# ruiminshen/yolo2-pytorch

Hardware: AMD Instinct MI355X
Metric: images/sec (416x416) train+detect, Darknet-19 YOLOv2: value = TRAIN step, batch 64 per GPU (configs[2]) at every N; detect (configs[1]) = roofline.detect_images_per_sec (higher is better)
Workload: dtype f32; 1 GPU; Darknet-19 YOLOv2 20-class train 416x416 batch-64/GPU: fwd + region loss + bwd + SGD (BASELINE configs[2]); classes=20, global_batch=64, parallelism=single GPU, weights=random-init seed 0 (bench_data.randomize)

## Files before the change

### include/yolo2_hip.h

```cpp
#ifndef YOLO2_HIP_H
#define YOLO2_HIP_H

#include <stdint.h>

#ifdef __cplusplus
extern "C" {
#endif

#define Y2_OK 0
#define Y2_EINVAL (-1)
#define Y2_EALIGN (-2)
#define Y2_ENOSUP (-3)

#define Y2_STATS_REPL 32

typedef void* y2_stream_t;

int y2_abi_version(void);
const char* y2_build_info(void);


int y2_pack_weight(const float* w, float* dst, int Cout, int Cin, int ksize, int mode, y2_stream_t stream);

#define Y2_PREP_FPROP 0
// ... 153 lines not shown
                       const float* gt_min, const float* gt_max, const long long* gt_cls, const uint8_t* gt_difficult,
                       int32_t B, int32_t M, int32_t G, int32_t C, float threshold, float min_union, uint8_t* tp, int32_t* cls_num);
int y2_collate_images_host(const uint8_t* src, const int64_t* offset, const int32_t* geom, const float* lut,
                           int32_t B, int32_t H, int32_t W, int32_t flags, float* out);
int y2_warp_affine_images_host(const uint8_t* src, const int64_t* src_offset, const int32_t* src_geom, const double* inv,
                               uint8_t* dst, const int64_t* dst_offset, const int32_t* dst_geom,
                               int32_t B, int32_t max_h, int32_t max_w, int32_t fill);
int y2_collate_jitter_images_host(const uint8_t* src, const int64_t* offset, const int32_t* geom, const int32_t* jitter, const uint8_t* hsv_tab,
                                  const float* lut, int32_t B, int32_t H, int32_t W, int32_t flags, float* out);

int y2_set_deterministic(int on, float* workspace, long long workspace_bytes);
int y2_get_deterministic(void);
int y2_colstats_det(const float* z, long long M, int32_t C, int32_t ld, double* stats, float* workspace, long long workspace_bytes, y2_stream_t stream);

int y2_prof_enable(int on);
int y2_prof_count(void);
int y2_prof_get(int i, char* name, int name_cap, float* ms, double* flops);
int y2_prof_set_tag(int tag);
int y2_prof_get_tag(int i);


int y2_conv_wgrad(const float* x, const float* dz, float* dw, int B, int H, int W, int Cin, int ldx, int Cout, int ldz,
                  int ksize, y2_stream_t stream);

int y2_conv_wgrad_ex(const float* x, const float* dz, float* dw, int B, int Hi, int Wi, int Cin, int ldx, int Cout, int ldz,
                     int ksize, int stride, int pad, y2_stream_t stream);

int y2_conv0_wgrad(const float* x_nchw, const float* dz, float* dw, int B, int H, int W, int Cin, int Cout, int ldz, y2_stream_t stream);

int y2_conv0_wgrad_fused(const float* x_nchw, const float* z, const float* scale, const float* shift, const float* mean, const float* invstd,
                         const float* gamma, float slope, const float* dy_pool, int32_t ldp, const double* sums, float* dw,
                         int32_t B, int32_t H, int32_t W, int32_t Cin, int32_t Cout, int32_t ldz, int32_t has_bn, y2_stream_t stream);

int y2_bn_finalize(const double* stats, double count, const float* gamma, const float* beta,
                   float* running_mean, float* running_var, float momentum, float eps,
                   float* scale, float* shift, float* mean, float* invstd, int C, long long* num_batches_tracked, y2_stream_t stream);

int y2_bn_act_fwd(const float* z, const float* scale, const float* shift, float slope, float* y, float* y_pool,
                  int B, int H, int W, int C, int ldz, int ldy, int coff, int ldp, int poff, int out_mode, y2_stream_t stream);

int y2_bn_act_bwd(const float* z, const float* scale, const float* shift, const float* mean, const float* invstd, const float* gamma,
                  float slope, const float* dy_full, int ldf, int foff, int fmode, const float* dy_pool, int ldp, int poff,
                  double* sums, float* dz, int ldd, int B, int H, int W, int C, int ldz, int has_bn, y2_stream_t stream);

int y2_bn_act_fwd_ex(const float* z, const float* scale, const float* shift, float slope, const float* residual, int ldr, float* y, float* y_pool,
                     int B, int H, int W, int C, int ldz, int ldy, int coff, int ldp, int poff, int out_mode, y2_stream_t stream);
int y2_bn_act_bwd_ex(const float* z, const float* scale, const float* shift, const float* mean, const float* invstd, const float* gamma,
                     float slope, const float* dy_full, int ldf, int foff, int fmode, const float* dy_pool, int ldp, int poff,
                     const float* dy_full2, int ld2, const float* residual, int ldr, float* dres, int lddr,
                     double* sums, float* dz, int ldd, int B, int H, int W, int C, int ldz, int has_bn, y2_stream_t stream);

long long y2_wino6_tiles(int32_t B, int32_t H, int32_t W);
int y2_bn_act_bwd_wino6(const float* z, const float* scale, const float* shift, const float* mean, const float* invstd, const float* gamma,
                        float slope, const float* dy_full, int ldf, int foff, double* sums, float* v6, float* m6, float* dz, int ldd,
                        int B, int H, int W, int C, int ldz, int has_bn, y2_stream_t stream);

int y2_maxpool_bwd(const float* x, const float* dy, const float* dy2, float* dx, int B, int H, int W, int C, int ldx, int ldy, int lddx,
                   int ksize, int stride, int pad, int pad_end, y2_stream_t stream);

int y2_colsum(const float* x, long long M, int C, int ld, double* out, y2_stream_t stream);
int y2_f64_to_f32(const double* src, float* dst, int n, double mul, y2_stream_t stream);

int y2_decode_bwd(const float* iou, const float* center_offset, const float* d_iou, const float* d_center_offset, const float* d_size_norm,
                  const float* d_logits, float* d_feature, int boxes, int C, y2_stream_t stream);

int y2_region_loss_fwd(const float* iou, const float* center_offset, const float* size_norm, const float* logits,
// ... 50 lines not shown
```

### yolo2-pytorch_amd/_hip.py

```python
import ctypes
import os
import subprocess

import torch

_HERE = os.path.dirname(os.path.abspath(__file__))
LIB_PATH = os.environ.get('Y2_LIB') or os.path.join(_HERE, 'csrc', 'libyolo2_hip.so')
_lib = None

c_int, c_float, c_void_p = ctypes.c_int, ctypes.c_float, ctypes.c_void_p


class ConvParams(ctypes.Structure):
    _fields_ = [('x', c_void_p), ('w', c_void_p), ('scale', c_void_p), ('shift', c_void_p),
                ('y', c_void_p), ('y_pool', c_void_p), ('stats', c_void_p),
                ('B', ctypes.c_int32), ('H', ctypes.c_int32), ('W', ctypes.c_int32),
                ('Cin', ctypes.c_int32), ('ldx', ctypes.c_int32), ('Cout', ctypes.c_int32), ('ksize', ctypes.c_int32),
                ('ldy', ctypes.c_int32), ('coff', ctypes.c_int32), ('ldp', ctypes.c_int32), ('poff', ctypes.c_int32),
                ('out_mode', ctypes.c_int32), ('slope', c_float), ('tile', ctypes.c_int32),
                ('workspace', c_void_p), ('workspace_bytes', ctypes.c_int64),
                ('residual', c_void_p), ('ldr', ctypes.c_int32), ('stride', ctypes.c_int32), ('pad_plus1', ctypes.c_int32),
                ('transposed', ctypes.c_int32), ('out_h', ctypes.c_int32), ('out_w', ctypes.c_int32), ('algo', ctypes.c_int32),
                ('w_plane', ctypes.c_int64)]

# ... 35 lines not shown
    'y2_gemm_split_f16': [c_void_p, c_void_p, c_void_p, ctypes.c_longlong, c_int, c_int, c_int, c_int, c_float, c_void_p],
    'y2_gemm_split': [c_void_p, c_void_p, c_void_p, ctypes.c_longlong, c_int, c_int, c_int, c_int, c_void_p],
    'y2_multi': [ctypes.POINTER(MultiItem), c_int, c_void_p],
    'y2_small_dot': [c_void_p, c_void_p, c_int, c_void_p, c_void_p],
    'y2_small_scale': [c_void_p, c_void_p, c_int, c_void_p, c_void_p],
    'y2_unpack_weight_grad': [c_void_p, c_void_p, c_int, c_int, c_int, c_void_p],
    'y2_bn_fold': [c_void_p, c_void_p, c_void_p, c_void_p, c_float, c_void_p, c_void_p, c_int, c_void_p],
    'y2_conv_fwd': [ctypes.POINTER(ConvParams), c_void_p],
    'y2_conv_fwd_workspace_bytes': [ctypes.POINTER(ConvParams)],
    'y2_wino_weight': [c_void_p, c_void_p, c_int, c_int, c_void_p],
    'y2_wino6_weight': [c_void_p, c_void_p, c_int, c_int, c_void_p],
    'y2_opt_sgd': [ctypes.POINTER(OptTensor), c_int, c_float, c_float, c_float, c_float, c_int, c_int, c_void_p],
    'y2_opt_adam': [ctypes.POINTER(OptTensor), c_int, c_float, c_float, c_float, c_float, c_float, c_int, c_void_p],
    'y2_opt_grad_sumsq': [ctypes.POINTER(OptTensor), c_int, c_void_p, c_void_p],
    'y2_opt_clip_grads': [ctypes.POINTER(OptTensor), c_int, c_void_p, c_float, c_void_p],
    'y2_wino_wgrad_workspace_bytes': [c_int, c_int, c_int, c_int, c_int],
    'y2_wino_wgrad_workspace_bytes_ex': [c_int, c_int, c_int, c_int, c_int, c_int],
    'y2_wino_wgrad': [c_void_p, c_void_p, c_void_p, c_int, c_int, c_int, c_int, c_int, c_int, c_int, c_void_p, c_void_p, ctypes.c_longlong, c_void_p],
    'y2_wino_wgrad_ex': [c_void_p, c_void_p, c_void_p, c_int, c_int, c_int, c_int, c_int, c_int, c_int, c_void_p, c_void_p, ctypes.c_longlong, c_int, c_void_p],
    'y2_conv_fwd_batch': [ctypes.POINTER(ConvParams), c_int, c_void_p],
    'y2_conv0_fwd': [c_void_p, c_void_p, c_void_p, c_void_p, c_void_p, c_void_p, c_void_p,
                     c_int, c_int, c_int, c_int, c_int, c_int, c_int, c_float, c_void_p],
    'y2_maxpool2_fwd': [c_void_p, c_void_p, c_int, c_int, c_int, c_int, c_int, c_int, c_void_p],
    'y2_maxpool_fwd': [c_void_p, c_void_p, c_int, c_int, c_int, c_int, c_int, c_int, c_int, c_int, c_int, c_int, c_void_p],
    'y2_nchw_to_nhwc': [c_void_p, c_void_p, c_int, c_int, c_int, c_int, c_int, c_void_p],
    'y2_decode': [c_void_p, c_void_p, c_int, c_int, c_int, c_int, c_int,
                  c_void_p, c_void_p, c_void_p, c_void_p, c_void_p, c_void_p, c_void_p, c_void_p, c_void_p],
    'y2_filter_visible': [c_void_p, c_void_p, c_int, c_int, c_int, c_int, c_float, c_void_p, c_void_p, c_void_p, c_void_p, c_void_p],
    'y2_iou_matrix': [c_void_p, c_void_p, c_void_p, c_void_p, c_int, c_int, c_int, c_float, c_int, c_void_p, c_void_p],
    'y2_iou_pair': [c_void_p, c_void_p, c_void_p, c_void_p, c_int, c_float, c_void_p, c_void_p],
    'y2_conv_wgrad': [c_void_p, c_void_p, c_void_p, c_int, c_int, c_int, c_int, c_int, c_int, c_int, c_int, c_void_p],
    'y2_conv_wgrad_ex': [c_void_p, c_void_p, c_void_p, c_int, c_int, c_int, c_int, c_int, c_int, c_int, c_int, c_int, c_int, c_void_p],
    'y2_conv0_wgrad_fused': [c_void_p] * 7 + [c_float, c_void_p, c_int, c_void_p, c_void_p] + [c_int] * 7 + [c_void_p],
    'y2_conv0_wgrad': [c_void_p, c_void_p, c_void_p, c_int, c_int, c_int, c_int, c_int, c_int, c_void_p],
    'y2_bn_finalize': [c_void_p, ctypes.c_double, c_void_p, c_void_p, c_void_p, c_void_p, c_float, c_float, c_void_p, c_void_p, c_void_p, c_void_p, c_int, c_void_p, c_void_p],
    'y2_bn_act_fwd': [c_void_p, c_void_p, c_void_p, c_float, c_void_p, c_void_p, c_int, c_int, c_int, c_int, c_int, c_int, c_int, c_int, c_int, c_int, c_void_p],
    'y2_bn_act_bwd': [c_void_p, c_void_p, c_void_p, c_void_p, c_void_p, c_void_p, c_float, c_void_p, c_int, c_int, c_int, c_void_p, c_int, c_int,
                      c_void_p, c_void_p, c_int, c_int, c_int, c_int, c_int, c_int, c_int, c_void_p],
    'y2_bn_act_fwd_ex': [c_void_p, c_void_p, c_void_p, c_float, c_void_p, c_int, c_void_p, c_void_p, c_int, c_int, c_int, c_int, c_int, c_int, c_int, c_int, c_int, c_int, c_void_p],
    'y2_bn_act_bwd_ex': [c_void_p, c_void_p, c_void_p, c_void_p, c_void_p, c_void_p, c_float, c_void_p, c_int, c_int, c_int, c_void_p, c_int, c_int,
                         c_void_p, c_int, c_void_p, c_int, c_void_p, c_int,
                         c_void_p, c_void_p, c_int, c_int, c_int, c_int, c_int, c_int, c_int, c_void_p],
    'y2_wino6_tiles': [c_int, c_int, c_int],
    'y2_bn_act_bwd_wino6': [c_void_p, c_void_p, c_void_p, c_void_p, c_void_p, c_void_p, c_float, c_void_p, c_int, c_int, c_void_p, c_void_p, c_void_p, c_void_p, c_int,
                            c_int, c_int, c_int, c_int, c_int, c_int, c_void_p],
    'y2_maxpool_bwd': [c_void_p, c_void_p, c_void_p, c_void_p, c_int, c_int, c_int, c_int, c_int, c_int, c_int, c_int, c_int, c_int, c_int, c_void_p],
    'y2_colsum': [c_void_p, ctypes.c_longlong, c_int, c_int, c_void_p, c_void_p],
    'y2_dwconv_fwd': [c_void_p, c_void_p, c_void_p, c_void_p, c_float, c_void_p, c_void_p, c_int, c_int, c_int, c_int, c_int, c_int, c_int, c_void_p],
    'y2_dwconv_dgrad': [c_void_p, c_void_p, c_void_p, c_int, c_int, c_int, c_int, c_int, c_int, c_int, c_void_p],
    'y2_dwconv_wgrad': [c_void_p, c_void_p, c_void_p, c_void_p, ctypes.c_longlong, c_int, c_int, c_int, c_int, c_int, c_int, c_int, c_void_p],
    'y2_dwconv_wgrad_workspace_bytes': [c_int, c_int, c_int, c_int, c_int],
    'y2_preact_conv1x1_fwd': [c_void_p, c_void_p, c_void_p, c_void_p, c_float, c_void_p, c_void_p, c_float, c_void_p, c_void_p] + [c_int] * 9 + [c_void_p],
    'y2_preact_fwd': [c_void_p, c_void_p, c_void_p, c_float, c_void_p] + [c_int] * 7 + [c_void_p],
    'y2_preact_bwd': [c_void_p, c_void_p, c_void_p, c_float, c_void_p, c_void_p, c_void_p, c_void_p, c_int, c_void_p, c_void_p, c_int, c_int] + [c_int] * 7 + [c_void_p],
    'y2_f64_to_f32': [c_void_p, c_void_p, c_int, ctypes.c_double, c_void_p],
    'y2_decode_bwd': [c_void_p, c_void_p, c_void_p, c_void_p, c_void_p, c_void_p, c_void_p, c_int, c_int, c_void_p],
    'y2_region_loss_fwd': [c_void_p] * 11 + [c_int] * 6 + [c_float] + [c_void_p] * 5 + [c_void_p],
    'y2_region_loss_finalize': [c_void_p, ctypes.c_double, c_int, c_void_p, c_void_p],
    'y2_region_loss_bwd': [c_void_p] * 9 + [c_int] * 6 + [c_float] + [c_void_p] * 5 + [c_void_p] * 4 + [c_void_p],
    'y2_nms_host': [c_void_p, c_void_p, c_void_p, c_void_p, c_void_p, c_int, c_int, c_float, c_int, c_void_p, c_void_p],
    'y2_iou_matrix_host': [c_void_p, c_void_p, c_void_p, c_void_p, c_int, c_int, c_int, c_float, c_int, c_void_p],
    'y2_iou_pair_host': [c_void_p, c_void_p, c_void_p, c_void_p, c_int, c_float, c_void_p],
    'y2_eval_match': [c_void_p] * 8 + [c_int, c_int, c_int, c_int, c_float, c_float, c_void_p, c_void_p, c_void_p],
    'y2_eval_match_host': [c_void_p] * 8 + [c_int, c_int, c_int, c_int, c_float, c_float, c_void_p, c_void_p],
    'y2_collate_images': [c_void_p] * 4 + [c_int, c_int, c_int, c_int, c_void_p, c_void_p],
    'y2_collate_images_host': [c_void_p] * 4 + [c_int, c_int, c_int, c_int, c_void_p],
    'y2_warp_affine_images': [c_void_p] * 7 + [c_int, c_int, c_int, c_int, c_void_p],
    'y2_warp_affine_images_host': [c_void_p] * 7 + [c_int, c_int, c_int, c_int],
    'y2_collate_jitter_images': [c_void_p] * 6 + [c_int, c_int, c_int, c_int, c_void_p, c_void_p],
    'y2_collate_jitter_images_host': [c_void_p] * 6 + [c_int, c_int, c_int, c_int, c_void_p],
    'y2_set_deterministic': [c_int, c_void_p, ctypes.c_longlong],
    'y2_get_deterministic': [],
    'y2_colstats_det': [c_void_p, ctypes.c_longlong, c_int, c_int, c_void_p, c_void_p, ctypes.c_longlong, c_void_p],
    'y2_prof_enable': [c_int],
    'y2_prof_count': [],
    'y2_prof_set_tag': [c_int],
    'y2_prof_get_tag': [c_int],
    'y2_prof_get': [c_int, ctypes.c_char_p, c_int, ctypes.POINTER(c_float), ctypes.POINTER(ctypes.c_double)],
    'y2_nms': [c_void_p, c_void_p, c_void_p, c_void_p, c_void_p, c_int, c_int, c_float, c_int, c_void_p, c_void_p, c_void_p, c_void_p],
}

STATS_REPL = 32

ERRORS = {-1: 'Y2_EINVAL (bad size / null pointer)', -2: 'Y2_EALIGN (unaligned pointer or stride)', -3: 'Y2_ENOSUP (unsupported combination)'}


class HipLibraryMissing(RuntimeError):
    pass


def build(verbose=False):
    out = subprocess.run(['bash', os.path.join(_HERE, 'csrc', 'build.sh')], capture_output=True, text=True)
    if verbose or out.returncode != 0:
        print(out.stdout + out.stderr)
    if out.returncode != 0:
        raise RuntimeError('building libyolo2_hip.so failed')
    return LIB_PATH


def lib():
    global _lib
    if _lib is None:
        if not os.path.exists(LIB_PATH):
            raise HipLibraryMissing('%s not found: run `python __graft_entry__.py build` (or yolo2-pytorch_amd/csrc/build.sh); '
                                    'the YOLOv2 hot path has no CPU/eager fallback' % LIB_PATH)
        l = ctypes.CDLL(LIB_PATH)
        for name, argtypes in SIGNATURES.items():
            fn = getattr(l, name)
            fn.argtypes = argtypes
            fn.restype = c_int
        l.y2_conv_fwd_workspace_bytes.restype = ctypes.c_longlong
        l.y2_wino_wgrad_workspace_bytes.restype = ctypes.c_longlong
        l.y2_wino6_tiles.restype = ctypes.c_longlong
        l.y2_dwconv_wgrad_workspace_bytes.restype = ctypes.c_longlong
        l.y2_wino_wgrad_workspace_bytes_ex.restype = ctypes.c_longlong
# ... 604 lines not shown
```

### yolo2-pytorch_amd/model/train_graph.py

```python
import collections
import ctypes
import os

import numpy as np
import torch
import torch.distributed as dist

import _hip
from model import train_oplist
from model._train_parts import BN_MOMENTUM, LEAKY, GradSink, StatsArena, _new, bn_params, cached_buf, prep_weights

BWD_STREAMS = int(os.environ.get('Y2_BWD_STREAMS', '2'))
_SIDE = {}


def _side_stream(dev):
    s = _SIDE.get(str(dev))
    if s is None:
        s = torch.cuda.Stream(device=dev)
        _SIDE[str(dev)] = s
    return s


GRAPH_FORK = {'1': True, '0': False}.get(os.environ.get('Y2_GRAPH_FORK', 'auto'), 'auto')
GRAD_F43 = os.environ.get('Y2_GRAD_F43', '1') != '0'
FUSE_WINO6 = os.environ.get('Y2_FUSE_WINO6', '1') != '0'
FUSE_CONV0 = os.environ.get('Y2_FUSE_CONV0', '1') != '0'
DEBUG_TAP = None

SYNC_POSITIVES = True

DP_TAG = '_y2_dp_reduce'


def _sum_over_ranks(t, reducer):
    return bool(reducer(t)) if reducer is not None else False


_WINO_CHUNK_BYTES = int(os.environ.get('Y2_WINO_CHUNK_MB', '4096')) << 20


OperandPruned = _hip.OperandMissing


def _problem(B, H, W, cin, ldx, cout, k, ldy, coff=0, ldp=0, out_mode=0, slope=1.0):
    p = _hip.ConvParams()
    p.x = p.y = 256
    p.B, p.H, p.W, p.Cin, p.ldx, p.Cout, p.ksize = B, H, W, cin, ldx, cout, k
    p.ldy, p.coff, p.ldp, p.poff, p.out_mode = ldy, coff, ldp, 0, out_mode
    p.slope, p.tile = slope, 0
    return p


def _f43_offered(eligible, cin, H, W):
    return bool(GRAD_F43 and eligible and cin >= 128 and H * W <= 52 * 52)


def _conv(L, st, x, wp, y, B, H, W, cin, ldx, cout, k, ldy, scale=None, shift=None, slope=1.0, stats=None, y_pool=None, ldp=0, coff=0, out_mode=0, keep_v=False, u=False,
          us=None, us_plane=0, grad=False, note=None, u_eligible=None, u6=None, choice=None, pre=None, problem=None):
    p = problem if problem is not None else _problem(B, H, W, cin, ldx, cout, k, ldy, coff, ldp, out_mode, slope)
# ... 285 lines not shown
    c_pt = eff[dnn.passthrough].cout
    c_l2 = eff[b2[-1][1]].cout
    cat = _new(dev, B, h, w, 4 * c_pt + c_l2)
    run_block('passthrough', dnn.passthrough, full_last, full_last.shape[-1], fh, fw, False, out_full=cat, out_ld=cat.shape[-1], out_off=0, out_mode=1)
    for i, (name, mod, pool) in enumerate(b2):
        if i == len(b2) - 1:
            blk, yf, yp = run_block(name, mod, cur, ld, h, w, False, out_full=cat, out_ld=cat.shape[-1], out_off=4 * c_pt)
        else:
            blk, yf, yp = run_block(name, mod, cur, ld, h, w, False)
            cur, ld = yf, blk.cout
    cur, ld = cat, cat.shape[-1]
    for i, (name, mod, pool) in enumerate(b3):
        blk, yf, yp = run_block(name, mod, cur, ld, h, w, False)
        cur, ld = yf, blk.cout
    if written:
        _hip.wrote(written)
    ctx.dnn = dnn
    ctx.blocks = blocks
    ctx.prepared = prepared
    ctx.prepared_key = dnn._train_cache[0] if (prepared and scope is None) else None
    ctx.scope = scope
    ctx.geom = (B, cin0, H, W, c_pt, c_l2)
    ctx.x = x
    ctx.frozen = frozen
    ctx.param_ids = [id(p) for p in params]
    L.y2_prof_set_tag(0)
    return cur


_Geo = collections.namedtuple('_Geo', 'H W cin cout k ldx first has_v padded ud_ok full pooled')
_Plan = collections.namedtuple('_Plan', 'wgrad zero final fuse0 fused6 problem')


def _routes(names, pools, n1, c_pt):
    idx = {name: i for i, name in enumerate(names)}
    out, full, pooled = [[] for _ in names], [None] * (len(names) - 1) + [0], [False] * len(names)
    for i, name in enumerate(names[1:], 1):
        if name == 'layers3.0':
            out[i] = [(idx['passthrough'], False, 0, 1), (i - 1, False, 4 * c_pt, 0)]
        elif name == 'passthrough':
            out[i] = [(n1 - 1, False, 0, 0)]
        elif i == n1 + 1:
            out[i] = [(n1 - 1, True, 0, 0)]
        else:
            out[i] = [(i - 1, pools[i - 1], 0, 0)]
    for j, is_pool, _, mode in sum(out, []):
        if is_pool:
            pooled[j] = True
        else:
            full[j] = mode
    return out, full, pooled


def _decide_bwd(geo, B, dev, need_dx=False):
    plans = []
    for g in geo:
        cop = (g.cout + 3) // 4 * 4
        if g.first:
            small = g.cin <= 3 and g.cout <= 64
            fuse0 = bool(FUSE_CONV0 and small and g.full is None and g.pooled and not (g.H & 1) and not (g.W & 15) and B * g.H * g.W * g.cout * 4 < 0xffff0000 and not need_dx)
            plans.append(_Plan(0, small, small, fuse0, None, None))
            continue
        wgrad = _hip.wgrad_choice(B, g.H, g.W, g.cin, g.ldx, cop, cop, g.k, g.has_v, dev)
        fused6 = problem = None
        if (FUSE_WINO6 and wgrad == 2 and g.k == 3 and g.ud_ok is not None and not g.pooled and g.full == 0 and cop == g.cout and not g.padded
                and DEBUG_TAP is None and not _hip.DETERMINISTIC and not _hip.split_mode()):
            problem = _problem(B, g.H, g.W, cop, cop, g.cin, g.k, g.cin)
            hit = _hip.autotune_conv(problem, dev, f43=True if _f43_offered(g.ud_ok, cop, g.H, g.W) else None, wino_eligible=g.ud_ok, peek=True)
            fused6 = tuple(hit) if (hit is not None and hit[0] == 6) else None
        plans.append(_Plan(wgrad, wgrad == 0, g.k == 1 and cop == g.cout and not g.padded, False, fused6, problem if fused6 else None))
    return plans


def _darknet_bwd(ctx, dout):
    L = _hip.lib()
    st = _hip.stream()
    dnn, blocks = ctx.dnn, ctx.blocks
    scope = getattr(ctx, 'scope', None)
    if ctx.prepared and scope is None and (getattr(dnn, '_train_cache', (None, None))[0] != ctx.prepared_key or ctx.prepared_key[:2] != (dout.device, dnn._weight_versions())):
        raise RuntimeError('model.yolo2: a convolution weight was modified (optimizer step, load_state_dict, in-place edit) between this forward and '
                           'its backward; the per-model GEMM operand buffers this graph was recorded against hold other weights now')
    B, cin0, H, W, c_pt, c_l2 = ctx.geom
    dev = dout.device
    dout = _hip.f32c(dout)
    sink = GradSink(dnn, dev)
    ready, dest, grads = sink.ready, sink.dest, sink.grads

    n = len(blocks)
    src_full, src_pool = [None] * (n - 1) + [(dout, blocks[n - 1].cout, 0, 0)], [None] * n
    routes, full, pooled = _routes([b.name for b in blocks], [b.pool for b in blocks], len(dnn._blocks()[0]), c_pt)
    need_dx = bool(getattr(ctx, 'need_dx', False))
    plans = _decide_bwd([_Geo(b.H, b.W, b.cin, b.cout, b.k, b.ldx, b.first, b.wino_v is not None, b.eff.padded,
                              ctx.prepared[b.mod]['ud_ok'] if (not b.first and b.mod in ctx.prepared) else None, full[i], pooled[i]) for i, b in enumerate(blocks)], B, str(dev), need_dx)
    order = list(range(n - 1, -1, -1))
    main = torch.cuda.current_stream(dev)
    side = _side_stream(dev) if (BWD_STREAMS > 1 and not _hip.DETERMINISTIC and (not torch.cuda.is_current_stream_capturing() or getattr(ctx, 'fork_ok', False))) else None
    late = []

    def join():
        for item in late:
            if item[2] is not None:
                main.wait_event(item[2])
                item[2] = None
    ctx.join = join
    affine_grads = []

    sums_arena = torch.empty(2 * sum(b.cout for b in blocks), dtype=torch.float64, device=dev)
    zero = [sums_arena]
    bufs = (dev, scope) if scope is not None else dnn.__dict__.setdefault('_train_bufs', (dev, {}))
    if bufs[0] != dev:
        bufs = dnn._train_bufs = (dev, {})
    wg, dzs = {}, {}
    for i in order:
        blk, plan = blocks[i], plans[i]
        cop = (blk.cout + 3) // 4 * 4
        weight = blk.mod.conv.weight
        if cop != blk.cout:
            dzs[i] = _new(dev, B, blk.H, blk.W, cop)
            zero.append(dzs[i])
        if blk.first:
            if plan.final:
                wg[i] = dest(weight) if not blk.eff.padded else _new(dev, blk.cout, blk.cin, 3, 3)
        elif blk.k == 1:
            wg[i] = dest(weight).view(-1) if plan.final else _new(dev, cop * blk.cin)
        else:
            wg[i] = cached_buf(bufs[1], (blk.name, 'dwp'), cop * blk.cin * blk.k * blk.k, dev)
        if plan.zero:
            zero.append(wg[i])
    _hip.multi([(_hip.MULTI_ZERO, t, None) for t in zero], st)
    sums_used = 0

    def flush_weight_grads(keep=0):
        while len(late) > keep:
            prm, g, evt, held = late.pop(0)
            if evt is not None:
                main.wait_event(evt)
            del held
            ready(prm, g)
    for i in order:
        blk, plan = blocks[i], plans[i]
        e = blk.eff
        L.y2_prof_set_tag(101 + i)
        h, w, cout, cin, k = blk.H, blk.W, blk.cout, blk.cin, blk.k
        sums = sums_arena[sums_used:sums_used + 2 * cout]
        sums_used += 2 * cout
        cop = (cout + 3) // 4 * 4
        sf, sp = src_full[i], src_pool[i]
        fuse0, fused6 = plan.fuse0, None
        if plan.fused6:
            T6 = int(L.y2_wino6_tiles(B, h, w))
            fused6 = (_new(dev, 36 * T6 * cout), _new(dev, 36 * T6 * cout))
        dz = None if (fuse0 or fused6) else (dzs[i] if i in dzs else _new(dev, B, h, w, cop))
        if DEBUG_TAP is not None:
            DEBUG_TAP(blk.name + ':in', blk.z, blk.shift, sf, sp)
        if fused6:
            _hip.check(L.y2_bn_act_bwd_wino6(_hip.ptr(blk.z), _hip.ptr(blk.scale), _hip.ptr(blk.shift), _hip.ptr(blk.mean), _hip.ptr(blk.invstd),
                                             _hip.ptr(e.gamma) if blk.has_bn else None, blk.slope, _hip.ptr(sf[0]), sf[1], sf[2], _hip.ptr(sums),
                                             _hip.ptr(fused6[0]), _hip.ptr(fused6[1]), None, 0, B, h, w, cout, cout,
                                             (2 if ctx.frozen else 1) if blk.has_bn else 0, st), 'y2_bn_act_bwd_wino6')
        else:
            _hip.check(L.y2_bn_act_bwd(_hip.ptr(blk.z), _hip.ptr(blk.scale), _hip.ptr(blk.shift), _hip.ptr(blk.mean), _hip.ptr(blk.invstd),
                                       _hip.ptr(e.gamma) if blk.has_bn else None, blk.slope,
                                       _hip.ptr(sf[0]) if sf else None, sf[1] if sf else 0, sf[2] if sf else 0, sf[3] if sf else 0,
                                       _hip.ptr(sp), cout, 0, _hip.ptr(sums), _hip.ptr(dz), cop, B, h, w, cout, cout,
                                       (2 if ctx.frozen else 1) if blk.has_bn else 0, st), 'y2_bn_act_bwd')
        if blk.has_bn:
            affine_grads.append((blk.mod.bn.bias, sums_used - 2 * cout, e.cout_r))
            affine_grads.append((blk.mod.bn.weight, sums_used - cout, e.cout_r))
        elif blk.mod.conv.bias is not None:
            affine_grads.append((blk.mod.conv.bias, sums_used - 2 * cout, e.cout_r))
        weight = blk.mod.conv.weight

        def real(dw):
            if not e.padded and cop == cout:
                return dw
            dw = dw[:e.cout_r]
            if e.cin != e.cin_r:
                dw = dw.index_select(1, torch.tensor(e.in_idx, dtype=torch.long, device=dev)) if e.in_idx is not None else dw[:, :e.cin_r].contiguous()
            return dw

        def weight_grad(st_w):
            if blk.first and fuse0:
                _hip.check(L.y2_conv0_wgrad_fused(_hip.ptr(ctx.x), _hip.ptr(blk.z), _hip.ptr(blk.scale), _hip.ptr(blk.shift), _hip.ptr(blk.mean), _hip.ptr(blk.invstd),
                                                  _hip.ptr(e.gamma) if blk.has_bn else None, blk.slope, _hip.ptr(sp), cout, _hip.ptr(sums), _hip.ptr(wg[i]),
                                                  B, h, w, cin, cout, cout, (2 if ctx.frozen else 1) if blk.has_bn else 0, st_w), 'y2_conv0_wgrad_fused')
                return real(wg[i])
            if blk.first and plan.final:
                _hip.check(L.y2_conv0_wgrad(_hip.ptr(ctx.x), _hip.ptr(dz), _hip.ptr(wg[i]), B, h, w, cin, cout, cop, st_w), 'y2_conv0_wgrad')
                return real(wg[i])
            if blk.first:
                x4 = torch.zeros(B, h, w, 4, dtype=torch.float32, device=dev)
                x4[..., :cin] = ctx.x.permute(0, 2, 3, 1)
                dwp = torch.zeros(cop * k * k * 4, dtype=torch.float32, device=dev)
                _hip.check(L.y2_conv_wgrad(_hip.ptr(x4), _hip.ptr(dz), _hip.ptr(dwp), B, h, w, 4, 4, cop, cop, k, st_w), 'y2_conv_wgrad')
                dw4 = _new(dev, cop, 4, k, k)
                _hip.check(L.y2_unpack_weight_grad(_hip.ptr(dwp), _hip.ptr(dw4), cop, 4, k, st_w), 'y2_unpack_weight_grad')
                return dw4[:e.cout_r, :cin].contiguous()
            tgt = wg[i]
            if plan.wgrad is None:
                _hip.multi([(_hip.MULTI_ZERO, tgt, None)], st_w)
            dw = None
            if k == 3:
                dw = dest(weight) if (cop == cout and not e.padded) else _new(dev, cop, cin, k, k)
            got = _hip.conv_wgrad(blk.x, fused6[1] if fused6 else dz, B, h, w, cin, blk.ldx, cop, cop, k, v=blk.wino_v, out=tgt, zeroed=plan.zero or plan.wgrad is None,
                                  native=dw, dz_pre=bool(fused6), choice=plan.wgrad)
            if plan.final:
                return tgt.view(cout, cin, 1, 1)
            if k == 1:
                return real(tgt.view(cop, cin, 1, 1))
            if got is not dw:
                _hip.check(L.y2_unpack_weight_grad(_hip.ptr(tgt), _hip.ptr(dw), cop, cin, k, st_w), 'y2_unpack_weight_grad')
            return real(dw)

        if side is not None and not e.padded and (not blk.first or plan.final):
# ... 17 lines not shown
            wd = _new(dev, wpad.numel())
            _hip.check(L.y2_pack_weight(_hip.ptr(wpad), _hip.ptr(wd), cop, cin4, k, 1, st), 'y2_pack_weight')
            dx4 = _new(dev, B, h, w, cin4)
            _conv(L, st, dz, wd, dx4, B, h, w, cop, cop, cin4, k, cin4)
            ctx_dx = dx4[..., :cin].permute(0, 3, 1, 2).contiguous()
            grads['__x__'] = ctx_dx
        if not blk.first:
            dx = _new(dev, B, h, w, cin)
            ready_ops = ctx.prepared.get(blk.mod)
            if ready_ops is not None:
                dg_split = ready_ops['uds'] if _hip.split_mode() == 'bf16' else None
                _conv(L, st, dz, ready_ops['wd'], dx, B, h, w, cop, cop, cin, k, cin, u=ready_ops['ud'], us=dg_split, us_plane=ready_ops['plane'], grad=True,
                      note=lambda kind, m=blk.mod: ctx.used.add((m, 'wd' if kind == 'w' else 'u6d' if kind == '6' else 'ud')), u_eligible=ready_ops['ud_ok'], u6=ready_ops.get('u6d'),
                      choice=plan.fused6, pre=fused6[0] if fused6 else None, problem=plan.problem)
            else:
                wsrc = e.w
                if cop != cout:
                    wpad = bufs[1].get((blk.name, 'wpad'))
                    if wpad is None or wpad.shape != (cop, cin, k, k):
                        wpad = bufs[1][(blk.name, 'wpad')] = torch.zeros(cop, cin, k, k, dtype=torch.float32, device=dev)
                    _hip.multi([(_hip.MULTI_COPY, wpad[:cout], wsrc)], st)
                    wsrc = wpad
                wd = _new(dev, wsrc.numel())
                _hip.check(L.y2_pack_weight(_hip.ptr(wsrc), _hip.ptr(wd), cop, cin, k, 1, st), 'y2_pack_weight')
                _conv(L, st, dz, wd, dx, B, h, w, cop, cop, cin, k, cin)
            if DEBUG_TAP is not None and dz is not None:
                DEBUG_TAP(blk.name, dz, dx, None, None)
            for j, to_pool, off, mode in routes[i]:
                if to_pool:
                    src_pool[j] = dx
                else:
                    src_full[j] = (dx, cin, off, mode)
        blk.z = None
    sink.hand_affine(sums_arena, affine_grads, st)
    flush_weight_grads()
    L.y2_prof_set_tag(0)
    out = [None, grads.get('__x__')]
    for pid in ctx.param_ids:
        out.append(grads.get(pid))
    ctx.blocks = None
    ctx.prepared = None
    ctx.join = None
    return tuple(out)


class DarknetTrainFn(torch.autograd.Function):
    @staticmethod
    def forward(ctx, dnn, x, *params):
        ctx.need_dx = x.requires_grad
        return _darknet_fwd(ctx, dnn, x, params, frozen=False)

    @staticmethod
    def backward(ctx, dout):
        return _darknet_bwd(ctx, dout)


class _Tape(object):
    need_dx = False
    saved_tensors = ()

    def save_for_backward(self, *tensors):
        self.saved_tensors = tensors

    def mark_non_differentiable(self, *tensors):
        pass

# ... 579 lines not shown
```

### yolo2-pytorch_amd/train.py

```python
import logging
import os

import numpy as np
import torch
import torch.distributed as dist
import torch.nn as nn

import model
import utils

BUCKET_BYTES = 25 * 1024 * 1024


_SCALES = {}


def norm_data(data, height, width, rows, cols, keys='yx_min, yx_max'):
    _data = {key: data[key] for key in data}
    t = _data[keys.split(', ')[0]]
    key = (rows / height, cols / width, str(t.device))
    scale = _SCALES.get(key)
    if scale is None:
        if len(_SCALES) > 256:
            _SCALES.clear()
# ... 455 lines not shown
            return False
        if not isinstance(inf, model.Inference) or not isinstance(dnn, (_yolo2.Darknet, _resnet.ResNet, _mobilenet.MobileNet, _densenet.DenseNet)) or not (inf.training and dnn.training):
            return False
        if _hip.DETERMINISTIC or train_graph.DEBUG_TAP is not None or not torch.is_grad_enabled() or torch.cuda.is_current_stream_capturing():
            return False
        if any(k not in data for k in ('yx_min', 'yx_max', 'cls')) or data['yx_min'].dim() != 3 or data['cls'].dim() not in (2, 3):
            return False
        ok = getattr(self, '_params_ok', None)
        if ok is not None:
            ps = self._params_seen
            if not all(p.requires_grad for p in ps) or self._param_ids(dnn) != self._params_ids_seen:
                self.plans.clear()
                ok = None
        if ok is None:
            ps = self._params_seen = list(dnn.parameters())
            self._mods_seen = [m for m in dnn.modules() if m._parameters]
            self._params_ids_seen = self._param_ids(dnn)
            ok = all(p.requires_grad and p.is_cuda and p.dtype == torch.float32 and p.is_contiguous() for p in ps)
            if ok and isinstance(dnn, _yolo2.Darknet) and not isinstance(dnn, _yolo2.Tiny):
                ok = train_graph._pad_layout(dnn) is None
            if ok and self.dp is not None:
                ok = all(id(p) in self.dp._where for p in ps) and len(ps) == len(self.dp._params)
            self._params_ok = ok
        return ok

    def step(self, data):
        import _hip
        from model import train_graph
        if not self.eligible(data):
            return None
        x, cls = data['tensor'], data['cls']
        n = data['yx_min'].shape[1]
        shape = (tuple(x.shape), tuple(cls.shape[2:]), cls.dim())
        tail = (_hip.tune_epoch(), _hip.WINOGRAD, _hip.split_mode(), _hip.FORCE_ALGO, train_graph.GRAD_F43, train_graph.FUSE_CONV0, str(x.device))
        mine = [k for k in self.plans if k[:3] == shape]
        for k in [k for k in mine if k[4:] != tail or not self.plans[k].valid()]:
            del self.plans[k]
            self._params_ok = None
        mine = [k for k in self.plans if k[:3] == shape]
        fit = sorted((k for k in mine if k[3] >= n), key=lambda k: k[3])
        if fit:
            key = fit[0]
            plan = self.plans[key]
            self.plans.move_to_end(key)
        else:
            npad = 16
            while npad < n:
                npad *= 2
            for k in mine:
                del self.plans[k]
            key = shape + (npad,) + tail
            plan = self._new_plan()
            plan._alloc(data, npad)
            plan.calls = self.warm.get(shape, 0)
            plan.used_last = self.used.get(shape)
            self.plans[key] = plan
            while len(self.plans) > self.MAX:
                self.plans.popitem(last=False)
        npad = key[3]
        self.warm[shape] = self.warm.get(shape, 0) + 1
        had_graph = plan.ops is not None
        out = plan.run(data, capture=GRAPH and not self.broken and shape not in self.eager_only)
        if plan.used_last:
            self.used[shape] = plan.used_last
        self.last = (npad, 'replay' if had_graph else ('capture' if plan.ops is not None else 'eager'))
        if plan.capture_error is not None and shape not in self.eager_only:
            e = plan.capture_error
# ... 54 lines not shown
```

Measured before the change: 2285 images/sec.

## Fuse conv0 BN/act backward and weight gradient into a single pass kernel

Adds a one-pass conv0 backward kernel. It recomputes the leaky activation and maxpool argmax from z, then accumulates the BN statistic sums together with two MFMA outer-product accumulators (raw and normalized-z terms). A finalize kernel applies the BN gradient correction algebraically to produce dw. This replaces the separate bn_act_bwd plus fused wgrad passes over the largest activation tensor, so z is read once instead of twice. In exchange it uses float atomics, which makes the result non-deterministic (the path is disabled in deterministic mode), and it adds an extra flush of weight gradients.

Measured after the change: 2293 images/sec, median of 6. Within noise of the previous version (+0.3%).

```diff
diff --git a/include/yolo2_hip.h b/include/yolo2_hip.h
--- a/include/yolo2_hip.h
+++ b/include/yolo2_hip.h
@@ -209,6 +209,11 @@
                          const float* gamma, float slope, const float* dy_pool, int32_t ldp, const double* sums, float* dw,
                          int32_t B, int32_t H, int32_t W, int32_t Cin, int32_t Cout, int32_t ldz, int32_t has_bn, y2_stream_t stream);
 
+#define Y2_CONV0_ONEPASS_ROWS 1024
+int y2_conv0_bwd_onepass(const float* x_nchw, const float* z, const float* scale, const float* shift, const float* mean, const float* invstd,
+                         const float* gamma, float slope, const float* dy_pool, int32_t ldp, float* acc, float* partial, double* sums, float* dw,
+                         int32_t B, int32_t H, int32_t W, int32_t Cin, int32_t Cout, int32_t ldz, int32_t has_bn, y2_stream_t stream);
+
 int y2_bn_finalize(const double* stats, double count, const float* gamma, const float* beta,
                    float* running_mean, float* running_var, float momentum, float eps,
                    float* scale, float* shift, float* mean, float* invstd, int C, long long* num_batches_tracked, y2_stream_t stream);
diff --git a/yolo2-pytorch_amd/_hip.py b/yolo2-pytorch_amd/_hip.py
--- a/yolo2-pytorch_amd/_hip.py
+++ b/yolo2-pytorch_amd/_hip.py
@@ -91,6 +91,7 @@
     'y2_conv_wgrad': [c_void_p, c_void_p, c_void_p, c_int, c_int, c_int, c_int, c_int, c_int, c_int, c_int, c_void_p],
     'y2_conv_wgrad_ex': [c_void_p, c_void_p, c_void_p, c_int, c_int, c_int, c_int, c_int, c_int, c_int, c_int, c_int, c_int, c_void_p],
     'y2_conv0_wgrad_fused': [c_void_p] * 7 + [c_float, c_void_p, c_int, c_void_p, c_void_p] + [c_int] * 7 + [c_void_p],
+    'y2_conv0_bwd_onepass': [c_void_p] * 7 + [c_float, c_void_p, c_int, c_void_p, c_void_p, c_void_p, c_void_p] + [c_int] * 7 + [c_void_p],
     'y2_conv0_wgrad': [c_void_p, c_void_p, c_void_p, c_int, c_int, c_int, c_int, c_int, c_int, c_void_p],
     'y2_bn_finalize': [c_void_p, ctypes.c_double, c_void_p, c_void_p, c_void_p, c_void_p, c_float, c_float, c_void_p, c_void_p, c_void_p, c_void_p, c_int, c_void_p, c_void_p],
     'y2_bn_act_fwd': [c_void_p, c_void_p, c_void_p, c_float, c_void_p, c_void_p, c_int, c_int, c_int, c_int, c_int, c_int, c_int, c_int, c_int, c_int, c_void_p],
@@ -140,6 +141,7 @@
 }
 
 STATS_REPL = 32
+CONV0_ONEPASS_ROWS = 1024
 
 ERRORS = {-1: 'Y2_EINVAL (bad size / null pointer)', -2: 'Y2_EALIGN (unaligned pointer or stride)', -3: 'Y2_ENOSUP (unsupported combination)'}
 
diff --git a/yolo2-pytorch_amd/csrc/conv0_bwd.hip b/yolo2-pytorch_amd/csrc/conv0_bwd.hip
--- /dev/null
+++ b/yolo2-pytorch_amd/csrc/conv0_bwd.hip
@@ -0,0 +1,213 @@
+#include "common.h"
+
+namespace {
+
+struct W0PArgs {
+    const float* x; const float* z; const float* scale; const float* shift; const float* mean; const float* invstd;
+    const float* dy_pool;
+    float* acc;
+    float* partial;
+    int B, H, W, Cin, Cout, ldz, ldp, pairs_total, has_bn;
+    unsigned z_bytes, p_bytes;
+    float slope;
+};
+
+template <int IB, bool BN>
+__global__ __launch_bounds__(256) void conv0_bwd_onepass_kernel(const W0PArgs a) {
+    __shared__ float red[4][IB * 32 * 33];
+    __shared__ float reds[4][2 * IB * 32 + 32];
+    const int t = threadIdx.x, lane = t & 63, wave = t >> 6;
+    const int l31 = lane & 31, half = lane >> 5;
+    const int K = a.Cin * 9;
+    const bool jok = l31 < K;
+    const int c = jok ? l31 / 9 : 0;
+    const int ky = jok ? (l31 % 9) / 3 : 0, kx = jok ? l31 % 3 : 0;
+    float sc[IB], sh[IB], mu[IB], is[IB];
+    bool cok[IB];
+#pragma unroll
+    for (int i = 0; i < IB; ++i) {
+        const int co = i * 32 + l31;
+        cok[i] = co < a.Cout;
+        const int cc = cok[i] ? co : 0;
+        sc[i] = a.scale ? a.scale[cc] : 1.f; sh[i] = a.shift ? a.shift[cc] : 0.f;
+        mu[i] = a.has_bn ? a.mean[cc] : 0.f; is[i] = a.has_bn ? a.invstd[cc] : 1.f;
+    }
+    f32x16 accA[IB], accB[IB];
+    float s1[IB], s2[IB], sx = 0.f;
+#pragma unroll
+    for (int i = 0; i < IB; ++i) {
+        s1[i] = 0.f; s2[i] = 0.f;
+#pragma unroll
+        for (int r = 0; r < 16; ++r) { accA[i][r] = 0.f; accB[i][r] = 0.f; }
+    }
+    const int wid = blockIdx.x * 4 + wave, nw = gridDim.x * 4;
+    const int Hh = a.H >> 1, Wh = a.W >> 1;
+    const __amdgpu_buffer_rsrc_t rz = __builtin_amdgcn_make_buffer_rsrc(const_cast<float*>(a.z), 0, a.z_bytes, 0x00020000);
+    const __amdgpu_buffer_rsrc_t rp = __builtin_amdgcn_make_buffer_rsrc(const_cast<float*>(a.dy_pool), 0, a.p_bytes, 0x00020000);
+    for (int pair = wid; pair < a.pairs_total; pair += nw) {
+        const int b = pair / Hh, r = pair - b * Hh;
+        const int y0 = 2 * r;
+        const int yy0 = y0 + ky - 1, yy1 = yy0 + 1;
+        const bool yok0 = jok && (unsigned)yy0 < (unsigned)a.H, yok1 = jok && (unsigned)yy1 < (unsigned)a.H;
+        const float* xr0 = a.x + (((size_t)b * a.Cin + c) * a.H + (yok0 ? yy0 : 0)) * a.W;
+        const float* xr1 = a.x + (((size_t)b * a.Cin + c) * a.H + (yok1 ? yy1 : 0)) * a.W;
+        const unsigned zrow = (unsigned)(((size_t)(b * a.H + y0) * a.W + half) * a.ldz * 4u) + (unsigned)l31 * 4u;
+        const unsigned prow = (unsigned)(((size_t)(b * Hh + r) * Wh) * a.ldp * 4u) + (unsigned)l31 * 4u;
+        const unsigned zstep = 2u * (unsigned)a.ldz * 4u, z1off = (unsigned)a.W * (unsigned)a.ldz * 4u, pstep = (unsigned)a.ldp * 4u;
+        for (int x0 = 0; x0 < a.W; x0 += 16) {
+            float z0[IB][8], z1[IB][8], dp[IB][8], bv0[8], bv1[8];
+            const unsigned zb = zrow + (unsigned)x0 * (unsigned)a.ldz * 4u, pb = prow + (unsigned)(x0 >> 1) * pstep;
+#pragma unroll
+            for (int s = 0; s < 8; ++s) {
+                const int px = x0 + 2 * s + half;
+#pragma unroll
+                for (int i = 0; i < IB; ++i) {
+                    z0[i][s] = __builtin_bit_cast(float, __builtin_amdgcn_raw_buffer_load_b32(rz, (int)(zb + i * 128u), (int)(s * zstep), 0));
+                    z1[i][s] = __builtin_bit_cast(float, __builtin_amdgcn_raw_buffer_load_b32(rz, (int)(zb + i * 128u), (int)(s * zstep + z1off), 0));
+                    dp[i][s] = __builtin_bit_cast(float, __builtin_amdgcn_raw_buffer_load_b32(rp, (int)(pb + i * 128u), (int)(s * pstep), 0));
+                }
+                const int xx = px + kx - 1;
+                const bool xok = px < a.W && (unsigned)xx < (unsigned)a.W;
+                bv0[s] = (xok && yok0) ? xr0[xx] : 0.f;
+                bv1[s] = (xok && yok1) ? xr1[xx] : 0.f;
+                sx += bv0[s] + bv1[s];
+            }
+#pragma unroll
+            for (int s = 0; s < 8; ++s)
+#pragma unroll
+                for (int i = 0; i < IB; ++i) {
+                    const float u0 = z0[i][s] * sc[i] + sh[i], u1 = z1[i][s] * sc[i] + sh[i];
+                    const float v0 = u0 > 0.f ? u0 : u0 * a.slope, v1 = u1 > 0.f ? u1 : u1 * a.slope;
+                    const float o0 = __shfl_xor(v0, 32), o1 = __shfl_xor(v1, 32);
+                    const float q0 = half ? o0 : v0, q1 = half ? v0 : o0, q2 = half ? o1 : v1, q3 = half ? v1 : o1;
+                    float best = q0; int arg = 0;
+                    if (q1 > best) { best = q1; arg = 1; }
+                    if (q2 > best) { best = q2; arg = 2; }
+                    if (q3 > best) { best = q3; arg = 3; }
+                    const bool ok = (x0 + 2 * s + half) < a.W && cok[i];
+                    const float g0 = (ok && arg == half) ? dp[i][s] : 0.f, g1 = (ok && arg == 2 + half) ? dp[i][s] : 0.f;
+                    const float ge0 = g0 * (u0 > 0.f ? 1.f : a.slope), ge1 = g1 * (u1 > 0.f ? 1.f : a.slope);
+                    const float zh0 = ok ? (z0[i][s] - mu[i]) * is[i] : 0.f, zh1 = ok ? (z1[i][s] - mu[i]) * is[i] : 0.f;
+                    s1[i] += ge0 + ge1;
+                    s2[i] += ge0 * zh0 + ge1 * zh1;
+                    accA[i] = __builtin_amdgcn_mfma_f32_32x32x2f32(ge0, bv0[s], accA[i], 0, 0, 0);
+                    accA[i] = __builtin_amdgcn_mfma_f32_32x32x2f32(ge1, bv1[s], accA[i], 0, 0, 0);
+                    if (BN) {
+                        accB[i] = __builtin_amdgcn_mfma_f32_32x32x2f32(zh0, bv0[s], accB[i], 0, 0, 0);
+                        accB[i] = __builtin_amdgcn_mfma_f32_32x32x2f32(zh1, bv1[s], accB[i], 0, 0, 0);
+                    }
+                }
+        }
+    }
+#pragma unroll
+    for (int i = 0; i < IB; ++i) {
+        s1[i] += __shfl_xor(s1[i], 32); s2[i] += __shfl_xor(s2[i], 32);
+    }
+    sx += __shfl_xor(sx, 32);
+    if (half == 0) {
+#pragma unroll
+        for (int i = 0; i < IB; ++i) { reds[wave][i * 32 + l31] = s1[i]; reds[wave][IB * 32 + i * 32 + l31] = s2[i]; }
+        reds[wave][2 * IB * 32 + l31] = sx;
+    }
+#pragma unroll
+    for (int m = 0; m < 2; ++m) {
+        if (m == 1 && !BN) break;
+        if (m == 1) __syncthreads();
+#pragma unroll
+        for (int i = 0; i < IB; ++i)
+#pragma unroll
+            for (int r = 0; r < 16; ++r) {
+                const int co = i * 32 + (r & 3) + 8 * (r >> 2) + 4 * half;
+                red[wave][co * 33 + l31] = m ? accB[i][r] : accA[i][r];
+            }
+        __syncthreads();
+        for (int e = t; e < IB * 32 * 32; e += 256) {
+            const int co = e >> 5, j = e & 31;
+            if (co < a.Cout && j < K)
+                atomicAdd(a.acc + ((size_t)m * a.Cout + co) * K + j, red[0][co * 33 + j] + red[1][co * 33 + j] + red[2][co * 33 + j] + red[3][co * 33 + j]);
+        }
+    }
+    if (t < 2 * IB * 32) {
+        const int m = t / (IB * 32), co = t - m * (IB * 32);
+        if (co < a.Cout) a.partial[(size_t)blockIdx.x * 2 * a.Cout + (size_t)m * a.Cout + co] = reds[0][t] + reds[1][t] + reds[2][t] + reds[3][t];
+    } else if (t < 2 * IB * 32 + 32) {
+        const int j = t - 2 * IB * 32;
+        if (j < K) atomicAdd(a.acc + (size_t)2 * a.Cout * K + j, reds[0][t] + reds[1][t] + reds[2][t] + reds[3][t]);
+    }
+}
+
+struct W0PFin {
+    const float* acc; const float* partial; const float* gamma; const float* invstd;
+    double* sums; float* dw;
+    int rows, Cin, Cout, has_bn;
+    double n;
+};
+
+__global__ __launch_bounds__(1024) void conv0_bwd_finalize_kernel(const W0PFin f) {
+    __shared__ double part[1024];
+    __shared__ double tot[128];
+    const int t = threadIdx.x;
+    const int n2 = 2 * f.Cout, K = 9 * f.Cin;
+    int cp = 2, sh = 1;
+    while (cp < n2) { cp <<= 1; ++sh; }
+    const int col = t & (cp - 1), lane = t >> sh, L = 1024 >> sh;
+    double s = 0.0;
+    if (col < n2)
+        for (int r = lane; r < f.rows; r += 16 * L) {
+            float v[16];
+#pragma unroll
+            for (int q = 0; q < 16; ++q) v[q] = (r + q * L < f.rows) ? f.partial[(size_t)(r + q * L) * n2 + col] : 0.f;
+#pragma unroll
+            for (int q = 0; q < 16; ++q) s += (double)v[q];
+        }
+    part[t] = s;
+    __syncthreads();
+    if (t < 128) {
+        double v = 0.0;
+        if (t < n2)
+            for (int l = 0; l < L; ++l) v += part[l * cp + t];
+        tot[t] = v;
+        if (t < n2) f.sums[t] = v;
+    }
+    __syncthreads();
+    const float* A = f.acc;
+    const float* Bh = f.acc + (size_t)f.Cout * K;
+    const float* Sx = f.acc + (size_t)2 * f.Cout * K;
+    for (int e = t; e < f.Cout * K; e += 1024) {
+        const int co = e / K, j = e - co * K;
+        double v = (double)A[e];
+        if (f.has_bn == 1) v -= (tot[co] / f.n) * (double)Sx[j] + (tot[f.Cout + co] / f.n) * (double)Bh[e];
+        const double gs = f.has_bn ? (double)f.gamma[co] * (double)f.invstd[co] : 1.0;
+        f.dw[e] = (float)(gs * v);
+    }
+}
+
+}
+
+extern "C" int y2_conv0_bwd_onepass(const float* x_nchw, const float* z, const float* scale, const float* shift, const float* mean, const float* invstd,
+                                    const float* gamma, float slope, const float* dy_pool, int ldp, float* acc, float* partial, double* sums, float* dw,
+                                    int B, int H, int W, int Cin, int Cout, int ldz, int has_bn, y2_stream_t stream) {
+    if (!x_nchw || !z || !dy_pool || !acc || !partial || !sums || !dw || B <= 0 || H <= 0 || W <= 0 || Cout <= 0 || ldz < Cout || ldp < Cout) return Y2_EINVAL;
+    if (has_bn < 0 || has_bn > 2 || (has_bn && (!mean || !invstd || !gamma))) return Y2_EINVAL;
+    if ((H & 1) || (W & 1)) return Y2_EINVAL;
+    if (Cin < 1 || Cin > 3 || Cout > 64 || (W & 15)) return Y2_ENOSUP;
+    if (y2_det.on) return Y2_ENOSUP;
+    const unsigned long long zb = (unsigned long long)B * H * W * ldz * 4ull, pb = (unsigned long long)B * (H / 2) * (W / 2) * ldp * 4ull;
+    if (zb >= 0xffff0000ull) return Y2_ENOSUP;
+    W0PArgs a;
+    a.z_bytes = (unsigned)zb; a.p_bytes = (unsigned)pb;
+    a.x = x_nchw; a.z = z; a.scale = scale; a.shift = shift; a.mean = mean; a.invstd = invstd; a.dy_pool = dy_pool; a.acc = acc; a.partial = partial;
+    a.B = B; a.H = H; a.W = W; a.Cin = Cin; a.Cout = Cout; a.ldz = ldz; a.ldp = ldp; a.pairs_total = B * (H / 2); a.has_bn = has_bn; a.slope = slope;
+    const int grid = a.pairs_total < 4 * Y2_CONV0_ONEPASS_ROWS ? y2_cdiv(a.pairs_total, 4) : Y2_CONV0_ONEPASS_ROWS;
+    const double flops = 2.0 * (double)B * H * W * 9 * Cin * Cout * (has_bn == 1 ? 2.0 : 1.0);
+    if (Cout <= 32 && has_bn == 1) Y2_LAUNCH("conv0_bwd_onepass_kernel", flops, (conv0_bwd_onepass_kernel<1, true>), dim3(grid), dim3(256), 0, y2_s(stream), a);
+    else if (Cout <= 32) Y2_LAUNCH("conv0_bwd_onepass_kernel", flops, (conv0_bwd_onepass_kernel<1, false>), dim3(grid), dim3(256), 0, y2_s(stream), a);
+    else if (has_bn == 1) Y2_LAUNCH("conv0_bwd_onepass_kernel", flops, (conv0_bwd_onepass_kernel<2, true>), dim3(grid), dim3(256), 0, y2_s(stream), a);
+    else Y2_LAUNCH("conv0_bwd_onepass_kernel", flops, (conv0_bwd_onepass_kernel<2, false>), dim3(grid), dim3(256), 0, y2_s(stream), a);
+    W0PFin f;
+    f.acc = acc; f.partial = partial; f.gamma = gamma; f.invstd = invstd; f.sums = sums; f.dw = dw;
+    f.rows = grid; f.Cin = Cin; f.Cout = Cout; f.has_bn = has_bn; f.n = (double)B * H * W;
+    Y2_LAUNCH("conv0_bwd_finalize_kernel", 0.0, conv0_bwd_finalize_kernel, dim3(1), dim3(1024), 0, y2_s(stream), f);
+    Y2_LAUNCH_CHECK();
+    return Y2_OK;
+}
diff --git a/yolo2-pytorch_amd/model/train_graph.py b/yolo2-pytorch_amd/model/train_graph.py
--- a/yolo2-pytorch_amd/model/train_graph.py
+++ b/yolo2-pytorch_amd/model/train_graph.py
@@ -26,6 +26,7 @@
 GRAD_F43 = os.environ.get('Y2_GRAD_F43', '1') != '0'
 FUSE_WINO6 = os.environ.get('Y2_FUSE_WINO6', '1') != '0'
 FUSE_CONV0 = os.environ.get('Y2_FUSE_CONV0', '1') != '0'
+CONV0_ONEPASS = os.environ.get('Y2_CONV0_ONEPASS', '1') != '0'
 DEBUG_TAP = None
 
 SYNC_POSITIVES = True
@@ -377,6 +378,10 @@
 _Plan = collections.namedtuple('_Plan', 'wgrad zero final fuse0 fused6 problem')
 
 
+class _Plans(list):
+    onepass = False
+
+
 def _routes(names, pools, n1, c_pt):
     idx = {name: i for i, name in enumerate(names)}
     out, full, pooled = [[] for _ in names], [None] * (len(names) - 1) + [0], [False] * len(names)
@@ -398,13 +403,14 @@
 
 
 def _decide_bwd(geo, B, dev, need_dx=False):
-    plans = []
+    plans = _Plans()
     for g in geo:
         cop = (g.cout + 3) // 4 * 4
         if g.first:
             small = g.cin <= 3 and g.cout <= 64
             fuse0 = bool(FUSE_CONV0 and small and g.full is None and g.pooled and not (g.H & 1) and not (g.W & 15) and B * g.H * g.W * g.cout * 4 < 0xffff0000 and not need_dx)
             plans.append(_Plan(0, small, small, fuse0, None, None))
+            plans.onepass = bool(fuse0 and CONV0_ONEPASS and not _hip.DETERMINISTIC and DEBUG_TAP is None)
             continue
         wgrad = _hip.wgrad_choice(B, g.H, g.W, g.cin, g.ldx, cop, cop, g.k, g.has_v, dev)
         fused6 = problem = None
@@ -470,7 +476,13 @@
             wg[i] = dest(weight).view(-1) if plan.final else _new(dev, cop * blk.cin)
         else:
             wg[i] = cached_buf(bufs[1], (blk.name, 'dwp'), cop * blk.cin * blk.k * blk.k, dev)
-        if plan.zero:
+        onepass = blk.first and plans.onepass
+        if onepass:
+            k0 = 9 * blk.cin
+            acc0 = cached_buf(bufs[1], (blk.name, 'onepass_acc'), (2 * blk.cout + 1) * k0, dev)
+            part0 = cached_buf(bufs[1], (blk.name, 'onepass_part'), _hip.CONV0_ONEPASS_ROWS * 2 * blk.cout, dev)
+            zero.append(acc0)
+        elif plan.zero:
             zero.append(wg[i])
     _hip.multi([(_hip.MULTI_ZERO, t, None) for t in zero], st)
     sums_used = 0
@@ -492,6 +504,7 @@
         cop = (cout + 3) // 4 * 4
         sf, sp = src_full[i], src_pool[i]
         fuse0, fused6 = plan.fuse0, None
+        onepass = blk.first and plans.onepass
         if plan.fused6:
             T6 = int(L.y2_wino6_tiles(B, h, w))
             fused6 = (_new(dev, 36 * T6 * cout), _new(dev, 36 * T6 * cout))
@@ -503,7 +516,7 @@
                                              _hip.ptr(e.gamma) if blk.has_bn else None, blk.slope, _hip.ptr(sf[0]), sf[1], sf[2], _hip.ptr(sums),
                                              _hip.ptr(fused6[0]), _hip.ptr(fused6[1]), None, 0, B, h, w, cout, cout,
                                              (2 if ctx.frozen else 1) if blk.has_bn else 0, st), 'y2_bn_act_bwd_wino6')
-        else:
+        elif not onepass:
             _hip.check(L.y2_bn_act_bwd(_hip.ptr(blk.z), _hip.ptr(blk.scale), _hip.ptr(blk.shift), _hip.ptr(blk.mean), _hip.ptr(blk.invstd),
                                        _hip.ptr(e.gamma) if blk.has_bn else None, blk.slope,
                                        _hip.ptr(sf[0]) if sf else None, sf[1] if sf else 0, sf[2] if sf else 0, sf[3] if sf else 0,
@@ -525,6 +538,11 @@
             return dw
 
         def weight_grad(st_w):
+            if onepass:
+                _hip.check(L.y2_conv0_bwd_onepass(_hip.ptr(ctx.x), _hip.ptr(blk.z), _hip.ptr(blk.scale), _hip.ptr(blk.shift), _hip.ptr(blk.mean), _hip.ptr(blk.invstd),
+                                                  _hip.ptr(e.gamma) if blk.has_bn else None, blk.slope, _hip.ptr(sp), cout, _hip.ptr(acc0), _hip.ptr(part0), _hip.ptr(sums),
+                                                  _hip.ptr(wg[i]), B, h, w, cin, cout, cout, (2 if ctx.frozen else 1) if blk.has_bn else 0, st_w), 'y2_conv0_bwd_onepass')
+                return real(wg[i])
             if blk.first and fuse0:
                 _hip.check(L.y2_conv0_wgrad_fused(_hip.ptr(ctx.x), _hip.ptr(blk.z), _hip.ptr(blk.scale), _hip.ptr(blk.shift), _hip.ptr(blk.mean), _hip.ptr(blk.invstd),
                                                   _hip.ptr(e.gamma) if blk.has_bn else None, blk.slope, _hip.ptr(sp), cout, _hip.ptr(sums), _hip.ptr(wg[i]),
@@ -608,6 +626,8 @@
                 else:
                     src_full[j] = (dx, cin, off, mode)
         blk.z = None
+    if plans.onepass:
+        flush_weight_grads()
     sink.hand_affine(sums_arena, affine_grads, st)
     flush_weight_grads()
     L.y2_prof_set_tag(0)
diff --git a/yolo2-pytorch_amd/train.py b/yolo2-pytorch_amd/train.py
--- a/yolo2-pytorch_amd/train.py
+++ b/yolo2-pytorch_amd/train.py
@@ -511,7 +511,7 @@
         x, cls = data['tensor'], data['cls']
         n = data['yx_min'].shape[1]
         shape = (tuple(x.shape), tuple(cls.shape[2:]), cls.dim())
-        tail = (_hip.tune_epoch(), _hip.WINOGRAD, _hip.split_mode(), _hip.FORCE_ALGO, train_graph.GRAD_F43, train_graph.FUSE_CONV0, str(x.device))
+        tail = (_hip.tune_epoch(), _hip.WINOGRAD, _hip.split_mode(), _hip.FORCE_ALGO, train_graph.GRAD_F43, train_graph.FUSE_CONV0, train_graph.CONV0_ONEPASS, str(x.device))
         mine = [k for k in self.plans if k[:3] == shape]
         for k in [k for k in mine if k[4:] != tail or not self.plans[k].valid()]:
             del self.plans[k]
```
